# KoonMing/KZG-Batch-Verification-Scheme

Hardware: AMD Instinct MI355X
Metric: batch-verifies/sec + G1 MSM pts/sec at n=2^20, BLS12-381; 1/2/4/8 GPU (higher is better)
Workload: dtype Montgomery Fp, 381-bit modular integer (radix-2^29 limbs in the bucket accumulation); 1 GPU; batch_verify (configs[2]): n=1048576 bls12_381 tuples per GPU, two G1 MSMs + 2-pairing check; curve=bls12_381, tuples_per_gpu=1048576, global_batch=1048576, pipeline_slots=16, parallelism=point-range shards

## Files before the change

kzg-batch-verification-scheme_amd/csrc/field29.hpp:

```cpp
#pragma once
#include "field.hpp"
#include <type_traits>
#include "params29_gen.hpp"

namespace kzgmi {

constexpr uint32_t M29 = (1u << 29) - 1;

template <class Cv>
using Fp29Of = std::conditional_t<Cv::ID == 0, Bls12_381Fp29, Bn254Fp29>;

template <class Q>
struct F29 {
  static constexpr int N = Q::N;
  uint32_t v[N];
  KZ_DEV static F29 zero() { F29 r; _Pragma("unroll") for (int i = 0; i < N; ++i) r.v[i] = 0; return r; }
  KZ_DEV static F29 from_const(const uint32_t (&c)[N]) {
    F29 r;
    _Pragma("unroll") for (int i = 0; i < N; ++i) r.v[i] = c[i];
    return r;
  }
};

KZ_DEV void mad29(uint64_t& acc, uint32_t a, uint32_t b) {
// ... 197 lines not shown
      r.v[i] = x & M29;
      c = x >> 29;
    } else {
      r.v[i] = x;
    }
  }
  return r;
}

template <class Q>
KZ_DEV F29<Q> sub3_29(const F29<Q>& a, const F29<Q>& s, const F29<Q>& t, const uint32_t (&C)[Q::N]) {
  F29<Q> r;
  uint32_t c = 0;
  _Pragma("unroll") for (int i = 0; i < Q::N; ++i) {
    const uint32_t x = (a.v[i] + C[i] + c) - (s.v[i] + t.v[i] + t.v[i]);
    if (i < Q::N - 1) {
      r.v[i] = x & M29;
      c = x >> 29;
    } else {
      r.v[i] = x;
    }
  }
  return r;
}

template <class Q>
KZ_DEV F29<Q> neg_lazy29(const F29<Q>& b, const uint32_t (&B)[Q::N]) {
  F29<Q> r;
  _Pragma("unroll") for (int i = 0; i < Q::N; ++i) r.v[i] = B[i] - b.v[i];
  return r;
}

template <class Q>
KZ_DEV F29<Q> add3_29(const F29<Q>& a, const F29<Q>& b, const F29<Q>& e) {
  F29<Q> r;
  uint32_t c = 0;
  _Pragma("unroll") for (int i = 0; i < Q::N; ++i) {
    const uint32_t x = a.v[i] + b.v[i] + e.v[i] + c;
    if (i < Q::N - 1) {
      r.v[i] = x & M29;
      c = x >> 29;
    } else {
      r.v[i] = x;
    }
  }
  return r;
}

template <class Q>
KZ_DEV bool is_zero29(const F29<Q>& a) {
  bool hit = false;
  _Pragma("unroll") for (int k = 0; k < Q::NKP; ++k) hit |= a.v[0] == Q::KP_LO[k];
  if (!hit) return false;
  for (int k = 0; k < Q::NKP; ++k) {
    uint32_t d = 0;
    for (int i = 0; i < Q::N; ++i) d |= a.v[i] ^ Q::KP[k][i];
    if (d == 0) return true;
  }
  return false;
}
template <class Q>
KZ_DEV bool is_zero29_mf(const F29<Q>& a) {
  constexpr uint32_t PINV = 0u - Q::INV;
  const uint32_t k = (a.v[0] * PINV) & M29;
  if (k >= (uint32_t)Q::NKP) return false;
  uint32_t d = 0;
  for (int i = 0; i < Q::N; ++i) d |= a.v[i] ^ Q::KP[k][i];
  return d == 0;
}

template <class Q>
KZ_DEV F29<Q> canon29(const F29<Q>& a) {
  F29<Q> d;
  int32_t c = 0;
  _Pragma("unroll") for (int i = 0; i < Q::N; ++i) {
    const int32_t x = (int32_t)a.v[i] - (int32_t)Q::MOD[i] + c;
    if (i < Q::N - 1) {
      d.v[i] = (uint32_t)x & M29;
      c = x >> 29;
    } else {
      d.v[i] = (uint32_t)x;
    }
  }
  const bool neg = (int32_t)d.v[Q::N - 1] < 0;
  F29<Q> r;
  _Pragma("unroll") for (int i = 0; i < Q::N; ++i) r.v[i] = neg ? a.v[i] : d.v[i];
  return r;
}

template <class Q, int NW>
KZ_DEV F29<Q> limbs29(const uint32_t (&w)[NW]) {
  F29<Q> r;
  _Pragma("unroll") for (int i = 0; i < Q::N; ++i) {
    const int bit = 29 * i, wi = bit >> 5, sh = bit & 31;
    const uint64_t lo = (wi < NW ? (uint64_t)w[wi] : 0) | (wi + 1 < NW ? (uint64_t)w[wi + 1] << 32 : 0);
    r.v[i] = (uint32_t)(lo >> sh) & (i < Q::N - 1 ? M29 : 0xffffffffu);
  }
  return r;
}
template <class Q, int NW>
KZ_DEV void words32(const F29<Q>& a, uint32_t (&w)[NW]) {
  _Pragma("unroll") for (int j = 0; j < NW; ++j) {
    const int bit = 32 * j, li = bit / 29, sh = bit % 29;
    uint64_t x = (uint64_t)a.v[li] >> sh;
    if (li + 1 < Q::N) x |= (uint64_t)a.v[li + 1] << (29 - sh);
    if (li + 2 < Q::N && 58 - sh < 32) x |= (uint64_t)a.v[li + 2] << (58 - sh);
    w[j] = (uint32_t)x;
  }
}

template <class Q, class P>
KZ_DEV F29<Q> fp_to29(const Fp<P>& a) {
  return mul29(limbs29<Q>(a.v), F29<Q>::from_const(Q::TO29));
}
template <class Q, class P>
KZ_DEV Fp<P> fp_from29(const F29<Q>& a) {
  Fp<P> r;
  words32<Q>(canon29(mul29(a, F29<Q>::from_const(Q::TO32))), r.v);
  return r;
}

}
// ... 1 lines not shown
```

kzg-batch-verification-scheme_amd/csrc/launch_msm.hip:

```cpp
#include "launch.hpp"

namespace kzgmi {

template <class F>
void with_wbits(int wbits, F&& f) {
  if (wbits == 13) f(std::integral_constant<int, 13>{});
  else f(std::integral_constant<int, WBITS>{});
}

template <class Cv>
void Launch<Cv>::sort(hipStream_t st, const TermList& tl, uint32_t nsets, const uint8_t* inf, uint32_t* digits,
                      uint32_t* coarse, uint64_t* ent, size_t emax, int sort_flags, uint32_t* off, uint32_t* cnt, uint32_t* total, uint32_t* sval,
                      uint32_t* skey, int wbits) {
  const bool force_split = (sort_flags & SORT_SPLIT) != 0;
  with_wbits(wbits, [&](auto wb) {
    constexpr int WB = decltype(wb)::value;
    const uint32_t nbins = nsets * Win<WB>::BINS;
    SetShift ss;
    const bool table = !(sort_flags & SORT_FULL_BINS) && set_shifts_host<WB>(tl, nsets, ss);
    uint32_t* ccnt = coarse;
    uint32_t* coff = coarse + nbins;
    uint32_t* ccur = coarse + 2 * nbins;
    (void)hipMemsetAsync(ccnt, 0, (size_t)nbins * 4, st);
    const uint32_t tiles = num_tiles_host(tl);
// ... 20 lines not shown
  });
}

template <class Cv>
void Launch<Cv>::accumulate(hipStream_t st, size_t nchunks, const uint32_t* total, const uint32_t* sval,
                            const uint32_t* skey, const uint32_t* off, const uint32_t* cnt, const AF* pts,
                            uint32_t* acc29, uint32_t nb, size_t acc_threads, uint32_t* next_chunk,
                            uint32_t* crowd, const uint32_t* lo, hipStream_t fix_st) {
  const unsigned blocks = grid_for(nchunks, 256);
  if (next_chunk && acc_threads && acc_threads < nchunks) {
    (void)hipMemsetAsync(next_chunk, 0, 4, st);
    k_accumulate<Cv><<<grid_for(acc_threads, 256), 256, 0, st>>>(total, sval, skey, off, cnt, pts, acc29, nb,
                                                                  (uint32_t)(blocks * 256u), next_chunk, lo, crowd);
  } else {
    k_accumulate<Cv><<<blocks, 256, 0, st>>>(total, sval, skey, off, cnt, pts, acc29, nb, 0u, nullptr, lo, crowd);
  }
  if (fix_st) fixup(fix_st, nchunks, total, skey, off, cnt, acc29, nb, crowd, lo);
}

template <class Cv>
void Launch<Cv>::fixup(hipStream_t st, size_t nchunks, const uint32_t* total, const uint32_t* skey, const uint32_t* off,
                       const uint32_t* cnt, uint32_t* acc29, uint32_t nb, uint32_t* crowd, const uint32_t* lo) {
  const unsigned blocks = grid_for(nchunks, 256);
  k_fixup<Cv><<<blocks, 256, 0, st>>>(total, skey, off, cnt, acc29, nb, crowd, lo);
  k_fixup_crowded<Cv><<<256, 256, 0, st>>>(crowd, acc29, nb, blocks * 256u);
}

template <class Cv>
void Launch<Cv>::row_items(hipStream_t st, const uint32_t* off, const uint32_t* cnt, uint32_t nb, uint32_t L, uint32_t* rowq,
                           uint32_t* items, uint32_t cap, uint32_t* cuts, uint32_t cut_cap) {
  (void)hipMemsetAsync(rowq, 0, (size_t)RQ_WORDS * 4, st);
  const unsigned blocks = grid_for(nb, ITEMS_BLOCK);
  k_items_hist<<<blocks, 256, 0, st>>>(cnt, nb, L, rowq);
  k_items_scan<<<1, 256, 0, st>>>(L, rowq);
  k_items_scatter<<<blocks, 256, 0, st>>>(off, cnt, nb, L, rowq, items, cap, cuts, cut_cap);
}

template <class Cv>
void Launch<Cv>::accumulate_rows(hipStream_t st, size_t threads, const uint32_t* sval, const AF* pts, uint32_t* acc29,
                                 uint32_t nb, uint32_t* rowq, const uint32_t* items, uint32_t cap, const uint32_t* cuts,
                                 uint32_t cut_cap) {
  k_accumulate_rows<Cv><<<grid_for(threads, 256), 256, 0, st>>>(rowq, items, cap, sval, pts, acc29);
  k_join_rows<Cv><<<64, 256, 0, st>>>(rowq, cuts, acc29, nb, cut_cap);
}

template <class Cv>
void Launch<Cv>::pts_to29(hipStream_t st, AF* pts, uint32_t n) {
  if (n) k_pts_to29<Cv><<<grid_for(n, 256), 256, 0, st>>>(pts, n);
}

template <class Cv>
void Launch<Cv>::reduce(hipStream_t st, uint32_t nsets, const uint32_t* cnt, const uint32_t* acc29, XY* R, XY* U,
                        XY* scratch, XY* winsum, int wbits, bool low_prio, int seg4_waves, int simds) {
  with_wbits(wbits, [&](auto wb) {
    constexpr int WB = decltype(wb)::value;
    const uint32_t nseg = nsets * Win<WB>::NSEG;
    const bool four = seg4_waves > 0 && (size_t)nseg * 4 <= (size_t)seg4_waves * simds * 64;
    auto go = [&](auto lp) {
      constexpr bool LP = decltype(lp)::value;
      if (four) k_reduce_segments4<Cv, LP><<<grid_for(4 * (size_t)nseg, 256), 256, 0, st>>>(nseg, cnt, acc29, R, U);
      else k_reduce_segments<Cv, LP><<<grid_for(2 * (size_t)nseg, 256), 256, 0, st>>>(nseg, cnt, acc29, R, U);
      k_reduce_bits<Cv, WB, LP><<<nsets * Win<WB>::RB_PARTS, 256, 0, st>>>(R, U, scratch);
      if (four) k_reduce_bits_finish<Cv, WB, LP, 4><<<nsets, 64, 0, st>>>(scratch, winsum);
      else k_reduce_bits_finish<Cv, WB, LP, 2><<<nsets, 64, 0, st>>>(scratch, winsum);
    };
    if (low_prio) go(std::true_type{});
    else go(std::false_type{});
// ... 52 lines not shown
```

kzg-batch-verification-scheme_amd/csrc/msm.hpp:

```cpp
#pragma once
#include "common.hpp"
#include "field29.hpp"
#include "lpfield.hpp"

namespace kzgmi {

constexpr int WBITS = 16;
constexpr int NBUCKETS = 1 << (WBITS - 1);
constexpr int ACC_CHUNK = 64;
constexpr int ACC_CHUNK_SMALL = 16;
constexpr size_t ACC_SMALL_ENTRIES = size_t(1) << 20;
constexpr int SEG = 16;
constexpr int MAX_CLASSES = 16;

struct TermClass {
  uint32_t count;
  uint32_t pt_base;
  uint32_t scal_words;
  uint32_t nwin;
  uint32_t set_base;
  uint32_t scal_stride;
  const uint32_t* scal;
  uint32_t win_off;
  uint32_t dig_base;
// ... 632 lines not shown
  uint32_t w[W29];
#pragma unroll
  for (int k = 0; k < N; ++k) {
    w[k] = a.x.v[k];
    w[N + k] = a.y.v[k];
    w[2 * N + k] = a.inf ? 0u : a.zz.v[k];
    w[3 * N + k] = a.zzz.v[k];
  }
  uint4* d4 = reinterpret_cast<uint4*>(acc29 + r * W29);
#pragma unroll
  for (int k = 0; k < W29 / 4; ++k) d4[k] = make_uint4(w[4 * k], w[4 * k + 1], w[4 * k + 2], w[4 * k + 3]);
}
template <class Q>
KZ_DEV X29<Q> x29_swap_pair(const X29<Q>& a) {
  X29<Q> o;
#pragma unroll
  for (int k = 0; k < Q::N; ++k) {
    o.x.v[k] = (uint32_t)__shfl_xor((int)a.x.v[k], 1);
    o.y.v[k] = (uint32_t)__shfl_xor((int)a.y.v[k], 1);
    o.zz.v[k] = (uint32_t)__shfl_xor((int)a.zz.v[k], 1);
    o.zzz.v[k] = (uint32_t)__shfl_xor((int)a.zzz.v[k], 1);
  }
  o.inf = __shfl_xor((int)a.inf, 1) != 0;
  return o;
}
template <class Cv, class Q>
KZ_DEV Xyzz<Cv> x29_to32(const X29<Q>& a) {
  using P = typename Cv::FpP;
  if (a.inf) return Xyzz<Cv>::inf();
  return {fp_from29<Q, P>(a.x), fp_from29<Q, P>(a.y), fp_from29<Q, P>(a.zz), fp_from29<Q, P>(a.zzz)};
}
template <class Cv>
constexpr bool kFusedSub = Cv::ID == 0;

template <class Q>
KZ_DEV X29<Q> x29_dbl(const X29<Q>& a) {
  using G = F29<Q>;
  if (a.inf) return a;
  const G U = add3_29(a.y, a.y, G::zero());
  const G V = sqr29(U);
  const G W = mul29(U, V);
  const G S = mul29(a.x, V);
  const G X2 = sqr29(a.x);
  const G M = add3_29(X2, X2, X2);
  X29<Q> o;
  o.x = sub29(sqr29(M), add3_29(S, S, G::zero()), Q::B4);
  o.y = mul2_29(M, sub29(S, o.x, Q::B8), W, sub29(G::zero(), a.y, Q::B16));
  o.zz = mul29(V, a.zz);
  o.zzz = mul29(W, a.zzz);
  o.inf = false;
  return o;
}

template <class Cv, class Q>
KZ_DEV X29<Q> x29_add(const X29<Q>& a, const X29<Q>& b) {
  using G = F29<Q>;
  if (a.inf) return b;
  if (b.inf) return a;
  const G U1 = mul29(a.x, b.zz), S1 = mul29(a.y, b.zzz);
  const G P = kFusedSub<Cv> ? mulsub29(b.x, a.zz, U1, Q::B2) : sub29(mul29(b.x, a.zz), U1, Q::B2);
  const G R = kFusedSub<Cv> ? mulsub29(b.y, a.zzz, S1, Q::B2) : sub29(mul29(b.y, a.zzz), S1, Q::B2);
  if (is_zero29(P)) {
    if (is_zero29(R)) return x29_dbl<Q>(a);
    return {G::zero(), G::zero(), G::zero(), G::zero(), true};
  }
  const G PP = sqr29(P);
// ... 315 lines not shown
constexpr uint32_t ROW_LEN_MAX = 256;
enum : uint32_t {
  RQ_NEXT = 0, RQ_NITEMS = 1, RQ_NCUT = 2, RQ_PIECES = 3, RQ_HIST = 4, RQ_CUR = RQ_HIST + ROW_LEN_MAX + 1,
  RQ_WORDS = RQ_CUR + ROW_LEN_MAX + 1
};

KZ_DEV void items_count(uint32_t* h, uint32_t c, uint32_t L) {
  if (c <= L) {
    atomicAdd(&h[c], 1u);
  } else {
    atomicAdd(&h[L], c / L);
    if (c % L) atomicAdd(&h[c % L], 1u);
  }
}

constexpr uint32_t ITEMS_PER_THREAD = 4, ITEMS_BLOCK = 256 * ITEMS_PER_THREAD;

static __global__ void __launch_bounds__(256) k_items_hist(const uint32_t* __restrict__ cnt, uint32_t nb, uint32_t L,
                                                           uint32_t* __restrict__ rowq) {
  __shared__ uint32_t h[ROW_LEN_MAX + 1];
  for (uint32_t t = threadIdx.x; t <= L; t += blockDim.x) h[t] = 0;
  __syncthreads();
#pragma unroll
  for (uint32_t k = 0; k < ITEMS_PER_THREAD; ++k) {
    const uint32_t b = blockIdx.x * ITEMS_BLOCK + k * 256 + threadIdx.x;
    const uint32_t c = b < nb ? cnt[b] : 0u;
    if (c) items_count(h, c, L);
  }
  __syncthreads();
  for (uint32_t t = threadIdx.x; t <= L; t += blockDim.x)
    if (h[t]) atomicAdd(&rowq[RQ_HIST + t], h[t]);
}

static __global__ void __launch_bounds__(256) k_items_scan(uint32_t L, uint32_t* __restrict__ rowq) {
  __shared__ uint32_t h[ROW_LEN_MAX + 1];
  for (uint32_t t = threadIdx.x; t <= L; t += blockDim.x) h[t] = t ? rowq[RQ_HIST + t] : 0u;
  __syncthreads();
  for (uint32_t t = threadIdx.x; t <= L; t += blockDim.x) {
    uint32_t before = 0;
    for (uint32_t l = t + 1; l <= L; ++l) before += h[l];
    rowq[RQ_CUR + t] = before;
    if (t == 0) rowq[RQ_NITEMS] = before;
  }
}

static __global__ void __launch_bounds__(256) k_items_scatter(const uint32_t* __restrict__ off,
                                                              const uint32_t* __restrict__ cnt, uint32_t nb, uint32_t L,
                                                              uint32_t* __restrict__ rowq, uint32_t* __restrict__ items,
                                                              uint32_t cap, uint32_t* __restrict__ cuts, uint32_t cut_cap) {
  __shared__ uint32_t h[ROW_LEN_MAX + 1], base[ROW_LEN_MAX + 1];
  for (uint32_t t = threadIdx.x; t <= L; t += blockDim.x) h[t] = 0;
  __syncthreads();
  uint32_t c[ITEMS_PER_THREAD], rank[ITEMS_PER_THREAD];
#pragma unroll
  for (uint32_t k = 0; k < ITEMS_PER_THREAD; ++k) {
    const uint32_t b = blockIdx.x * ITEMS_BLOCK + k * 256 + threadIdx.x;
    c[k] = b < nb ? cnt[b] : 0u;
    rank[k] = c[k] && c[k] <= L ? atomicAdd(&h[c[k]], 1u) : 0u;
  }
  __syncthreads();
  for (uint32_t t = threadIdx.x; t <= L; t += blockDim.x)
    if (h[t]) base[t] = atomicAdd(&rowq[RQ_CUR + t], h[t]);
  __syncthreads();
  auto put = [&](uint32_t pos, uint32_t rec, uint32_t first, uint32_t len) {
    if (pos >= cap) return;
    items[pos] = rec;
    items[cap + pos] = first;
    items[2 * (size_t)cap + pos] = len;
  };
#pragma unroll
  for (uint32_t k = 0; k < ITEMS_PER_THREAD; ++k) {
    const uint32_t b = blockIdx.x * ITEMS_BLOCK + k * 256 + threadIdx.x;
    if (!c[k]) continue;
    const uint32_t o = off[b];
    if (c[k] <= L) {
      put(base[c[k]] + rank[k], b, o, c[k]);
      continue;
    }
    const uint32_t np = (c[k] + L - 1) / L;
    const uint32_t slot = atomicAdd(&rowq[RQ_PIECES], np);
    const uint32_t line = atomicAdd(&rowq[RQ_NCUT], 1u);
    if (line >= cut_cap) continue;
    cuts[3 * (size_t)line] = b;
    cuts[3 * (size_t)line + 1] = slot;
    cuts[3 * (size_t)line + 2] = np;
    for (uint32_t j = 0; j < np; ++j) {
      const uint32_t len = min(L, c[k] - j * L);
      put(atomicAdd(&rowq[RQ_CUR + len], 1u), nb + slot + j, o + j * L, len);
    }
  }
}

template <class Cv>
KZ_DEV void acc_row29(uint32_t first, uint32_t len, uint32_t rec, const uint32_t* __restrict__ sorted_val,
                      const uint32_t* __restrict__ pts29, uint32_t* __restrict__ acc29) {
  using Q = Fp29Of<Cv>;
  using G = F29<Q>;
  constexpr int N = Q::N, W29 = kW29<Q>;
  __shared__ uint32_t s_zz[N][256], s_zzz[N][256];
  __shared__ uint4 s_vq[256];
  const uint32_t tx = threadIdx.x;
  auto ld = [tx](uint32_t (&a)[N][256]) {
    asm volatile("" ::: "memory");
    G r;
    _Pragma("unroll") for (int k = 0; k < N; ++k) r.v[k] = a[k][tx];
    return r;
  };
  auto st = [tx](uint32_t (&a)[N][256], const G& v) {
    _Pragma("unroll") for (int k = 0; k < N; ++k) a[k][tx] = v.v[k];
    asm volatile("" ::: "memory");
  };
  auto put = [](uint32_t* d, const G& a) {
    if constexpr (N % 2 == 0) {
      _Pragma("unroll") for (int k = 0; k < N / 2; ++k) reinterpret_cast<uint2*>(d)[k] = make_uint2(a.v[2 * k], a.v[2 * k + 1]);
    } else {
      _Pragma("unroll") for (int k = 0; k < N; ++k) d[k] = a.v[k];
    }
  };
  auto load_q = [&](uint32_t v, G& qx, G& qy) {
    load_pt29<Cv>(reinterpret_cast<const Affine<Cv>*>(pts29) + sv_point(v), qx, qy);
    if (v & 1) qy = sub29(G::zero(), qy, Q::ACC_NEG);
  };
  auto set_one = [&]() {
    const G one = one_literals<Q>(std::make_integer_sequence<int, N / 2>{});
    st(s_zz, one);
    st(s_zzz, one);
  };
  uint4* const vq_wave = &s_vq[tx & ~63u];
  const uint32_t end = first + len;
  uint32_t e = first;
  G x, y;
  bool inf = false;
  load_q(sorted_val[e], x, y);
  set_one();
  ++e;
  for (;;) {
    bool dbl = false;
    __builtin_amdgcn_global_load_lds(reinterpret_cast<const uint4*>(sorted_val + (e & ~3u)), vq_wave, 16, 0, 0);
    for (; e < end; ++e) {
      const uint32_t j = e & 3u;
      uint32_t lane;
      asm volatile("v_mbcnt_lo_u32_b32 %0, -1, 0\n\tv_mbcnt_hi_u32_b32 %0, -1, %0" : "=v"(lane));
      const uint32_t v = reinterpret_cast<const uint32_t*>(&s_vq[(tx & ~63u) + lane])[j];
      if (j == 3) {
        __builtin_amdgcn_s_waitcnt(0xc07f);
        __builtin_amdgcn_global_load_lds(reinterpret_cast<const uint4*>(sorted_val + e + 1), vq_wave, 16, 0, 0);
      }
      G qx, qy;
      load_q(v, qx, qy);
      if (inf) {
        x = qx;
        y = qy;
        set_one();
        inf = false;
        continue;
      }
      const G P = kFusedSub<Cv> ? mulsub29(qx, ld(s_zz), x, Q::ACC_P) : sub29(mul29(qx, ld(s_zz)), x, Q::ACC_P);
      const G R = kFusedSub<Cv> ? mulsub29(qy, ld(s_zzz), y, Q::ACC_R) : sub29(mul29(qy, ld(s_zzz)), y, Q::ACC_R);
      if (is_zero29_mf(P)) {
        if (is_zero29_mf(R)) {
          dbl = true;
          break;
        }
        inf = true;
        continue;
      }
      const G PP = sqr29(P);
      const G PPP = mul29(P, PP);
      st(s_zz, mul29(ld(s_zz), PP));
      st(s_zzz, mul29(ld(s_zzz), PPP));
      const G Q2 = mul29(x, PP);
      const G X3 = kFusedSub<Cv> ? sqrsub3_29(R, PPP, Q2, Q::ACC_X3) : sub3_29(sqr29(R), PPP, Q2, Q::ACC_X3);
      y = mul2_29(R, sub29(Q2, X3, Q::ACC_QX), y, neg_lazy29(PPP, Q::ACC_PPP));
      x = X3;
    }
    if (!dbl) break;
    G qx, qy;
    load_q(sorted_val[e], qx, qy);
    asm volatile("" ::: "memory");
    const Xy29<Q> d = dbl_affine29<Q>(qx, qy, &s_zz[0][tx], &s_zzz[0][tx]);
    asm volatile("" ::: "memory");
    x = d.x;
    y = d.y;
    ++e;
  }
  uint32_t* d = acc29 + (size_t)rec * W29;
  put(d, x);
  put(d + N, y);
  put(d + 2 * N, inf ? G::zero() : ld(s_zz));
  put(d + 3 * N, ld(s_zzz));
}

template <class Cv>
__global__ void __launch_bounds__(256) __attribute__((amdgpu_waves_per_eu(kAccWaves<Cv>))) k_accumulate_rows(
    uint32_t* __restrict__ rowq, const uint32_t* __restrict__ items, uint32_t cap,
    const uint32_t* __restrict__ sorted_val, const Affine<Cv>* __restrict__ pts, uint32_t* __restrict__ acc29) {
  const uint32_t nitems = rowq[RQ_NITEMS];
  const uint32_t lane = threadIdx.x & 63u;
  for (;;) {
    uint32_t row = 0;
    if (lane == 0) row = atomicAdd(&rowq[RQ_NEXT], 1u);
    row = __shfl(row, 0);
    if ((uint64_t)row * 64 >= nitems) break;
    const uint32_t i = row * 64 + lane;
    if (i < nitems)
      acc_row29<Cv>(items[cap + i], items[2 * (size_t)cap + i], items[i], sorted_val,
                    reinterpret_cast<const uint32_t*>(pts), acc29);
  }
}

template <class Cv>
// ... 318 lines not shown
```

kzg-batch-verification-scheme_amd/csrc/params29_gen.hpp:

```cpp
#pragma once
#include <cstdint>

namespace kzgmi {

struct Bls12_381Fp29 {
  static constexpr int N = 14;
  static constexpr uint32_t MOD[N] = {0x1fffaaabu, 0xff7ffffu, 0x14ffffeeu, 0x17fffd62u, 0xf6241eau, 0x9507b58u, 0xafd9cc3u, 0x109e70a2u, 0x1764774bu, 0x121a5d66u, 0x12c6e9edu, 0x12ffcd34u, 0x111ea3u, 0xdu};
  static constexpr uint32_t INV = 0xfffcfffdu;
  static constexpr uint32_t ONE[N] = {0x3a9fb84u, 0xba00690u, 0x71288f1u, 0xf59bcc5u, 0x126cb614u, 0x585bf36u, 0x1b85ac3du, 0x1cf856fau, 0x1891ecbdu, 0x1a7eec05u, 0x155a88f0u, 0x741ac6du, 0x1317c30fu, 0x9u};
  static constexpr uint32_t TO29[N] = {0x1fddebbdu, 0x1a4f5474u, 0x291f399u, 0x14d03b3cu, 0xf6cad2cu, 0x1b4cabcau, 0x1592827cu, 0x21c6ac7u, 0x1ec52a84u, 0x16fd5ec4u, 0xc960da6u, 0xfd2af6bu, 0x13263591u, 0xbu};
  static constexpr uint32_t TO32[N] = {0x2fffdu, 0x10480000u, 0x300009du, 0x8001788u, 0x158baebfu, 0xc2ba9e3u, 0x1d157d22u, 0xa6e0a4au, 0xd77ce58u, 0x1d12b763u, 0x1701c6a5u, 0x1501c926u, 0x1f65ec3fu, 0xau};
  static constexpr uint32_t R2[N] = {0x15bef7aeu, 0x1031cd0eu, 0x2dd93e8u, 0x9226323u, 0xe6e2cd2u, 0x11684daau, 0x1170e5dbu, 0x88e25b1u, 0x1b366399u, 0x1c536f47u, 0xd1f9cbcu, 0x278b67fu, 0x1ea66a2bu, 0xcu};
  static constexpr uint32_t BCURVE[N] = {0xea898bau, 0xe901a40u, 0x124a23e8u, 0xd66f84fu, 0xaee547cu, 0x3760629u, 0x181b776eu, 0x12a47aa6u, 0x137ec460u, 0x5c6f549u, 0xfdc4fe8u, 0x1707174du, 0xc3ccef5u, 0xcu};
  static constexpr uint32_t B1[N] = {0x3fffaaabu, 0x2ff7fffeu, 0x34ffffedu, 0x37fffd61u, 0x2f6241e9u, 0x29507b57u, 0x2afd9cc2u, 0x309e70a1u, 0x3764774au, 0x321a5d65u, 0x32c6e9ecu, 0x32ffcd33u, 0x20111ea2u, 0xcu};
  static constexpr uint32_t B2[N] = {0x3fff5556u, 0x3feffffeu, 0x29ffffdbu, 0x2ffffac4u, 0x3ec483d4u, 0x32a0f6afu, 0x35fb3985u, 0x213ce143u, 0x2ec8ee96u, 0x2434baccu, 0x258dd3dau, 0x25ff9a68u, 0x20223d46u, 0x19u};
  static constexpr uint32_t B4[N] = {0x3ffeaaacu, 0x3fdffffeu, 0x33ffffb8u, 0x3ffff589u, 0x3d8907a9u, 0x2541ed60u, 0x2bf6730cu, 0x2279c288u, 0x3d91dd2du, 0x28697599u, 0x2b1ba7b5u, 0x2bff34d1u, 0x20447a8du, 0x33u};
  static constexpr uint32_t B8[N] = {0x3ffd5558u, 0x3fbffffeu, 0x27ffff72u, 0x3fffeb14u, 0x3b120f54u, 0x2a83dac2u, 0x37ece619u, 0x24f38511u, 0x3b23ba5bu, 0x30d2eb34u, 0x36374f6bu, 0x37fe69a3u, 0x2088f51bu, 0x67u};
  static constexpr uint32_t B16[N] = {0x3ffaaab0u, 0x3f7ffffeu, 0x2ffffee6u, 0x3fffd629u, 0x36241eaau, 0x3507b586u, 0x2fd9cc33u, 0x29e70a24u, 0x364774b7u, 0x21a5d66au, 0x2c6e9ed8u, 0x2ffcd348u, 0x2111ea38u, 0xcfu};
  static constexpr uint32_t B32[N] = {0x3ff55560u, 0x3efffffeu, 0x3ffffdceu, 0x3fffac53u, 0x2c483d56u, 0x2a0f6b0eu, 0x3fb39868u, 0x33ce1449u, 0x2c8ee96fu, 0x234bacd6u, 0x38dd3db1u, 0x3ff9a691u, 0x2223d471u, 0x19fu};
  static constexpr uint32_t B64[N] = {0x3feaaac0u, 0x3dfffffeu, 0x3ffffb9eu, 0x3fff58a8u, 0x38907aaeu, 0x341ed61du, 0x3f6730d1u, 0x279c2894u, 0x391dd2e0u, 0x269759adu, 0x31ba7b63u, 0x3ff34d24u, 0x2447a8e4u, 0x33fu};
  static constexpr uint32_t C4[N] = {0x7ffeaaacu, 0x7fdffffcu, 0x73ffffb6u, 0x7ffff587u, 0x7d8907a7u, 0x6541ed5eu, 0x6bf6730au, 0x6279c286u, 0x7d91dd2bu, 0x68697597u, 0x6b1ba7b3u, 0x6bff34cfu, 0x60447a8bu, 0x31u};
  static constexpr uint32_t C8[N] = {0x7ffd5558u, 0x7fbffffcu, 0x67ffff70u, 0x7fffeb12u, 0x7b120f52u, 0x6a83dac0u, 0x77ece617u, 0x64f3850fu, 0x7b23ba59u, 0x70d2eb32u, 0x76374f69u, 0x77fe69a1u, 0x6088f519u, 0x65u};
  static constexpr const uint32_t (&ACC_NEG)[N] = B8;
  static constexpr const uint32_t (&ACC_P)[N] = B16;
  static constexpr const uint32_t (&ACC_R)[N] = B16;
  static constexpr const uint32_t (&ACC_X3)[N] = C8;
  static constexpr const uint32_t (&ACC_QX)[N] = B16;
  static constexpr const uint32_t (&ACC_PPP)[N] = B8;
  static constexpr const uint32_t (&DBL_X)[N] = B8;
  static constexpr const uint32_t (&DBL_QX)[N] = B16;
  static constexpr const uint32_t (&DBL_Y)[N] = B8;
  static constexpr const uint32_t (&ACC_X3_B)[N] = B8;
  static constexpr int NKP = 20;
  static constexpr uint32_t KP_LO[NKP] = {0x0u, 0x1fffaaabu, 0x1fff5556u, 0x1fff0001u, 0x1ffeaaacu, 0x1ffe5557u, 0x1ffe0002u, 0x1ffdaaadu, 0x1ffd5558u, 0x1ffd0003u, 0x1ffcaaaeu, 0x1ffc5559u, 0x1ffc0004u, 0x1ffbaaafu, 0x1ffb555au, 0x1ffb0005u, 0x1ffaaab0u, 0x1ffa555bu, 0x1ffa0006u, 0x1ff9aab1u};
  static constexpr uint32_t KP[NKP][N] = {{0x0u, 0x0u, 0x0u, 0x0u, 0x0u, 0x0u, 0x0u, 0x0u, 0x0u, 0x0u, 0x0u, 0x0u, 0x0u, 0x0u}, {0x1fffaaabu, 0xff7ffffu, 0x14ffffeeu, 0x17fffd62u, 0xf6241eau, 0x9507b58u, 0xafd9cc3u, 0x109e70a2u, 0x1764774bu, 0x121a5d66u, 0x12c6e9edu, 0x12ffcd34u, 0x111ea3u, 0xdu}, {0x1fff5556u, 0x1fefffffu, 0x9ffffdcu, 0xffffac5u, 0x1ec483d5u, 0x12a0f6b0u, 0x15fb3986u, 0x13ce144u, 0xec8ee97u, 0x434bacdu, 0x58dd3dbu, 0x5ff9a69u, 0x223d47u, 0x1au}, {0x1fff0001u, 0xfe7ffffu, 0x1effffcbu, 0x7fff827u, 0xe26c5c0u, 0x1bf17209u, 0xf8d649u, 0x11db51e7u, 0x62d65e2u, 0x164f1834u, 0x1854bdc8u, 0x18ff679du, 0x335beau, 0x27u}, {0x1ffeaaacu, 0x1fdfffffu, 0x13ffffb9u, 0x1ffff58au, 0x1d8907aau, 0x541ed61u, 0xbf6730du, 0x279c289u, 0x1d91dd2eu, 0x869759au, 0xb1ba7b6u, 0xbff34d2u, 0x447a8eu, 0x34u}, {0x1ffe5557u, 0xfd7ffffu, 0x8ffffa8u, 0x17fff2edu, 0xceb4995u, 0xe9268bau, 0x16f40fd0u, 0x1318332bu, 0x14f65479u, 0x1a83d301u, 0x1de291a3u, 0x1eff0206u, 0x559931u, 0x41u}, {0x1ffe0002u, 0x1fcfffffu, 0x1dffff96u, 0xffff04fu, 0x1c4d8b80u, 0x17e2e412u, 0x1f1ac93u, 0x3b6a3ceu, 0xc5acbc5u, 0xc9e3068u, 0x10a97b91u, 0x11fecf3bu, 0x66b7d5u, 0x4eu}, {0x1ffdaaadu, 0xfc7ffffu, 0x12ffff85u, 0x7ffedb2u, 0xbafcd6bu, 0x1335f6bu, 0xcef4957u, 0x14551470u, 0x3bf4310u, 0x1eb88dcfu, 0x370657eu, 0x4fe9c70u, 0x77d679u, 0x5bu}, {0x1ffd5558u, 0x1fbfffffu, 0x7ffff73u, 0x1fffeb15u, 0x1b120f55u, 0xa83dac3u, 0x17ece61au, 0x4f38512u, 0x1b23ba5cu, 0x10d2eb35u, 0x16374f6cu, 0x17fe69a4u, 0x88f51cu, 0x68u}, {0x1ffd0003u, 0xfb7ffffu, 0x1cffff62u, 0x17ffe877u, 0xa745140u, 0x13d4561cu, 0x2ea82ddu, 0x1591f5b5u, 0x128831a7u, 0x2ed489cu, 0x8fe395au, 0xafe36d9u, 0x9a13c0u, 0x75u}, {0x1ffcaaaeu, 0x1fafffffu, 0x11ffff50u, 0xfffe5dau, 0x19d6932bu, 0x1d24d174u, 0xde81fa0u, 0x6306657u, 0x9eca8f3u, 0x1507a603u, 0x1bc52347u, 0x1dfe040du, 0xab3263u, 0x82u}, {0x1ffc5559u, 0xfa7ffffu, 0x6ffff3fu, 0x7ffe33du, 0x938d516u, 0x6754ccdu, 0x18e5bc64u, 0x16ced6f9u, 0x151203eu, 0x722036au, 0xe8c0d35u, 0x10fdd142u, 0xbc5107u, 0x8fu}, {0x1ffc0004u, 0x1f9fffffu, 0x1bffff2du, 0x1fffe09fu, 0x189b1700u, 0xfc5c825u, 0x3e35927u, 0x76d479cu, 0x18b5978au, 0x193c60d0u, 0x152f722u, 0x3fd9e77u, 0xcd6fabu, 0x9cu}, {0x1ffbaaafu, 0xf97ffffu, 0x10ffff1cu, 0x17ffde02u, 0x7fd58ebu, 0x1916437eu, 0xee0f5eau, 0x180bb83eu, 0x101a0ed5u, 0xb56be37u, 0x1419e110u, 0x16fd6babu, 0xde8e4eu, 0xa9u}, {0x1ffb555au, 0x1f8fffffu, 0x5ffff0au, 0xfffdb65u, 0x175f9ad6u, 0x266bed6u, 0x19de92aeu, 0x8aa28e0u, 0x77e8621u, 0x1d711b9eu, 0x6e0cafdu, 0x9fd38e0u, 0xefacf2u, 0xb6u}, {0x1ffb0005u, 0xf87ffffu, 0x1afffef9u, 0x7ffd8c7u, 0x6c1dcc1u, 0xbb73a2fu, 0x4dc2f71u, 0x19489983u, 0x1ee2fd6cu, 0xf8b7904u, 0x19a7b4ebu, 0x1cfd0614u, 0x100cb95u, 0xc3u}, {0x1ffaaab0u, 0x1f7fffffu, 0xffffee7u, 0x1fffd62au, 0x16241eabu, 0x1507b587u, 0xfd9cc34u, 0x9e70a25u, 0x164774b8u, 0x1a5d66bu, 0xc6e9ed9u, 0xffcd349u, 0x111ea39u, 0xd0u}, {0x1ffa555bu, 0xf77ffffu, 0x4fffed6u, 0x17ffd38du, 0x5866096u, 0x1e5830e0u, 0x1ad768f7u, 0x1a857ac7u, 0xdabec03u, 0x13c033d2u, 0x1f3588c6u, 0x2fca07du, 0x12308ddu, 0xddu}, {0x1ffa0006u, 0x1f6fffffu, 0x19fffec4u, 0xfffd0efu, 0x14e8a281u, 0x7a8ac38u, 0x5d505bbu, 0xb23eb6au, 0x510634fu, 0x5da9139u, 0x11fc72b4u, 0x15fc6db2u, 0x1342780u, 0xeau}, {0x1ff9aab1u, 0xf67ffffu, 0xefffeb3u, 0x7ffce52u, 0x44ae46cu, 0x10f92791u, 0x10d2a27eu, 0x1bc25c0cu, 0x1c74da9au, 0x17f4ee9fu, 0x4c35ca1u, 0x8fc3ae7u, 0x1454624u, 0xf7u}};
};

struct Bn254Fp29 {
  static constexpr int N = 9;
  static constexpr uint32_t MOD[N] = {0x187cfd47u, 0x10460b6u, 0x1c72a34fu, 0x2d522d0u, 0x1585d978u, 0x2db40c0u, 0xa6e141u, 0xe5c2634u, 0x30644eu};
  static constexpr uint32_t INV = 0xe4866389u;
  static constexpr uint32_t ONE[N] = {0x157ccc21u, 0x141c2758u, 0x185230d3u, 0x14c0419u, 0xaa36fb9u, 0x1d4240ceu, 0x11d54c07u, 0x52ac7a8u, 0xdc836u};
  static constexpr uint32_t TO29[N] = {0x13349ca1u, 0x1a5d84a8u, 0xa3e5cacu, 0x100249e0u, 0x12b951e8u, 0xe92d304u, 0x14cb95b3u, 0x41b9d3du, 0x58003u};
  static constexpr uint32_t TO32[N] = {0x58f0d9du, 0x1aea1c6eu, 0x11c2cf74u, 0x11d651ebu, 0x1462c0a7u, 0x11b7bc3cu, 0x1cbd99bau, 0x183340fbu, 0xe0a77u};
  static constexpr uint32_t R2[N] = {0x59bac10u, 0xd1503a3u, 0x18016b8u, 0x10ab0ca8u, 0x2632639u, 0x2c0169fu, 0x169bfd53u, 0x11869d4cu, 0x2a11a6u};
  static constexpr uint32_t BCURVE[N] = {0x766463u, 0x1c54760au, 0x8f6927au, 0x3e40c4du, 0x1fea4f2bu, 0x17c6c26au, 0x157fe417u, 0xf8056f9u, 0x2958a2u};
  static constexpr uint32_t B1[N] = {0x387cfd47u, 0x210460b5u, 0x3c72a34eu, 0x22d522cfu, 0x3585d977u, 0x22db40bfu, 0x20a6e140u, 0x2e5c2633u, 0x30644du};
  static constexpr uint32_t B2[N] = {0x30f9fa8eu, 0x2208c16cu, 0x38e5469du, 0x25aa45a0u, 0x2b0bb2efu, 0x25b68180u, 0x214dc281u, 0x3cb84c67u, 0x60c89bu};
  static constexpr uint32_t B4[N] = {0x21f3f51cu, 0x241182dau, 0x31ca8d3bu, 0x2b548b42u, 0x361765dfu, 0x2b6d0301u, 0x229b8503u, 0x397098cfu, 0xc19138u};
  static constexpr uint32_t B8[N] = {0x23e7ea38u, 0x282305b5u, 0x23951a77u, 0x36a91686u, 0x2c2ecbbfu, 0x36da0604u, 0x25370a07u, 0x32e1319fu, 0x1832272u};
  static constexpr uint32_t B16[N] = {0x27cfd470u, 0x30460b6bu, 0x272a34efu, 0x2d522d0du, 0x385d9780u, 0x2db40c09u, 0x2a6e1410u, 0x25c2633fu, 0x30644e6u};
  static constexpr uint32_t B32[N] = {0x2f9fa8e0u, 0x208c16d7u, 0x2e5469e0u, 0x3aa45a1bu, 0x30bb2f01u, 0x3b681814u, 0x34dc2821u, 0x2b84c67fu, 0x60c89cdu};
  static constexpr uint32_t B64[N] = {0x3f3f51c0u, 0x21182dafu, 0x3ca8d3c1u, 0x3548b437u, 0x21765e04u, 0x36d0302au, 0x29b85044u, 0x37098d00u, 0xc19139bu};
  static constexpr uint32_t C4[N] = {0x61f3f51cu, 0x641182d8u, 0x71ca8d39u, 0x6b548b40u, 0x761765ddu, 0x6b6d02ffu, 0x629b8501u, 0x797098cdu, 0xc19136u};
  static constexpr uint32_t C8[N] = {0x63e7ea38u, 0x682305b3u, 0x63951a75u, 0x76a91684u, 0x6c2ecbbdu, 0x76da0602u, 0x65370a05u, 0x72e1319du, 0x1832270u};
  static constexpr const uint32_t (&ACC_NEG)[N] = B2;
  static constexpr const uint32_t (&ACC_P)[N] = B8;
  static constexpr const uint32_t (&ACC_R)[N] = B4;
  static constexpr const uint32_t (&ACC_X3)[N] = C4;
  static constexpr const uint32_t (&ACC_QX)[N] = B8;
  static constexpr const uint32_t (&ACC_PPP)[N] = B2;
  static constexpr const uint32_t (&DBL_X)[N] = B4;
  static constexpr const uint32_t (&DBL_QX)[N] = B8;
  static constexpr const uint32_t (&DBL_Y)[N] = B2;
  static constexpr const uint32_t (&ACC_X3_B)[N] = B4;
// ... 7 lines not shown
```

Before: 199.7 batch-verifies/s (n=1048576 tuples per GPU per batch).

## Peel first bucket addition, use lazy negation, fold item scan into scatter

In BLS12-381 bucket row accumulation, the first two points of a row are now added with a specialised affine+affine step. It is guarded by range checks on the top limbs and a wave-wide ballot, so the generic mixed add and the set_one store are skipped when the inputs are safe. Point negation in the main loop uses a lazy unreduced form, normalised only when it is loaded into an infinity accumulator. The separate single-block k_items_scan launch is removed: every scatter block recomputes the suffix sums in shared memory and adds them to its atomic offsets. This trades redundant per-block scan work and extra range-check logic for one fewer kernel launch and less field arithmetic.

```diff
diff --git a/kzg-batch-verification-scheme_amd/csrc/field29.hpp b/kzg-batch-verification-scheme_amd/csrc/field29.hpp
--- a/kzg-batch-verification-scheme_amd/csrc/field29.hpp
+++ b/kzg-batch-verification-scheme_amd/csrc/field29.hpp
@@ -253,6 +253,22 @@
 }
 
 template <class Q>
+KZ_DEV F29<Q> norm29(const F29<Q>& a) {
+  F29<Q> r;
+  uint32_t c = 0;
+  _Pragma("unroll") for (int i = 0; i < Q::N; ++i) {
+    const uint32_t x = a.v[i] + c;
+    if (i < Q::N - 1) {
+      r.v[i] = x & M29;
+      c = x >> 29;
+    } else {
+      r.v[i] = x;
+    }
+  }
+  return r;
+}
+
+template <class Q>
 KZ_DEV F29<Q> add3_29(const F29<Q>& a, const F29<Q>& b, const F29<Q>& e) {
   F29<Q> r;
   uint32_t c = 0;
@@ -309,6 +325,15 @@
   return r;
 }
 
+template <class Q>
+KZ_DEV bool peel_ok29(const F29<Q>& v) {
+  constexpr int N = Q::N;
+  const uint32_t t1 = v.v[N - 1], t0 = v.v[N - 2];
+  const bool lo = (t1 != 0) | (t0 >= Q::PEEL_LO);
+  const bool hi = (t1 < Q::MOD[N - 1]) | ((t1 == Q::MOD[N - 1]) & (t0 < Q::MOD[N - 2]));
+  return lo & hi;
+}
+
 template <class Q, int NW>
 KZ_DEV F29<Q> limbs29(const uint32_t (&w)[NW]) {
   F29<Q> r;
diff --git a/kzg-batch-verification-scheme_amd/csrc/launch_msm.hip b/kzg-batch-verification-scheme_amd/csrc/launch_msm.hip
--- a/kzg-batch-verification-scheme_amd/csrc/launch_msm.hip
+++ b/kzg-batch-verification-scheme_amd/csrc/launch_msm.hip
@@ -76,7 +76,6 @@
   (void)hipMemsetAsync(rowq, 0, (size_t)RQ_WORDS * 4, st);
   const unsigned blocks = grid_for(nb, ITEMS_BLOCK);
   k_items_hist<<<blocks, 256, 0, st>>>(cnt, nb, L, rowq);
-  k_items_scan<<<1, 256, 0, st>>>(L, rowq);
   k_items_scatter<<<blocks, 256, 0, st>>>(off, cnt, nb, L, rowq, items, cap, cuts, cut_cap);
 }
 
diff --git a/kzg-batch-verification-scheme_amd/csrc/msm.hpp b/kzg-batch-verification-scheme_amd/csrc/msm.hpp
--- a/kzg-batch-verification-scheme_amd/csrc/msm.hpp
+++ b/kzg-batch-verification-scheme_amd/csrc/msm.hpp
@@ -688,6 +688,8 @@
 }
 template <class Cv>
 constexpr bool kFusedSub = Cv::ID == 0;
+template <class Cv>
+constexpr bool kPeelFirst = Cv::ID == 0;
 
 template <class Q>
 KZ_DEV X29<Q> x29_dbl(const X29<Q>& a) {
@@ -1069,25 +1071,22 @@
     if (h[t]) atomicAdd(&rowq[RQ_HIST + t], h[t]);
 }
 
-static __global__ void __launch_bounds__(256) k_items_scan(uint32_t L, uint32_t* __restrict__ rowq) {
-  __shared__ uint32_t h[ROW_LEN_MAX + 1];
-  for (uint32_t t = threadIdx.x; t <= L; t += blockDim.x) h[t] = t ? rowq[RQ_HIST + t] : 0u;
-  __syncthreads();
-  for (uint32_t t = threadIdx.x; t <= L; t += blockDim.x) {
-    uint32_t before = 0;
-    for (uint32_t l = t + 1; l <= L; ++l) before += h[l];
-    rowq[RQ_CUR + t] = before;
-    if (t == 0) rowq[RQ_NITEMS] = before;
-  }
-}
-
 static __global__ void __launch_bounds__(256) k_items_scatter(const uint32_t* __restrict__ off,
                                                               const uint32_t* __restrict__ cnt, uint32_t nb, uint32_t L,
                                                               uint32_t* __restrict__ rowq, uint32_t* __restrict__ items,
                                                               uint32_t cap, uint32_t* __restrict__ cuts, uint32_t cut_cap) {
-  __shared__ uint32_t h[ROW_LEN_MAX + 1], base[ROW_LEN_MAX + 1];
-  for (uint32_t t = threadIdx.x; t <= L; t += blockDim.x) h[t] = 0;
-  __syncthreads();
+  __shared__ uint32_t h[ROW_LEN_MAX + 1], base[ROW_LEN_MAX + 1], all[ROW_LEN_MAX + 1], before[ROW_LEN_MAX + 1];
+  for (uint32_t t = threadIdx.x; t <= L; t += blockDim.x) {
+    h[t] = 0;
+    all[t] = t ? rowq[RQ_HIST + t] : 0u;
+  }
+  __syncthreads();
+  for (uint32_t t = threadIdx.x; t <= L; t += blockDim.x) {
+    uint32_t s = 0;
+    for (uint32_t l = t + 1; l <= L; ++l) s += all[l];
+    before[t] = s;
+    if (t == 0 && blockIdx.x == 0) rowq[RQ_NITEMS] = s;
+  }
   uint32_t c[ITEMS_PER_THREAD], rank[ITEMS_PER_THREAD];
 #pragma unroll
   for (uint32_t k = 0; k < ITEMS_PER_THREAD; ++k) {
@@ -1097,7 +1096,7 @@
   }
   __syncthreads();
   for (uint32_t t = threadIdx.x; t <= L; t += blockDim.x)
-    if (h[t]) base[t] = atomicAdd(&rowq[RQ_CUR + t], h[t]);
+    if (h[t]) base[t] = before[t] + atomicAdd(&rowq[RQ_CUR + t], h[t]);
   __syncthreads();
   auto put = [&](uint32_t pos, uint32_t rec, uint32_t first, uint32_t len) {
     if (pos >= cap) return;
@@ -1123,7 +1122,7 @@
     cuts[3 * (size_t)line + 2] = np;
     for (uint32_t j = 0; j < np; ++j) {
       const uint32_t len = min(L, c[k] - j * L);
-      put(atomicAdd(&rowq[RQ_CUR + len], 1u), nb + slot + j, o + j * L, len);
+      put(before[len] + atomicAdd(&rowq[RQ_CUR + len], 1u), nb + slot + j, o + j * L, len);
     }
   }
 }
@@ -1154,10 +1153,15 @@
       _Pragma("unroll") for (int k = 0; k < N; ++k) d[k] = a.v[k];
     }
   };
-  auto load_q = [&](uint32_t v, G& qx, G& qy) {
+  auto load_q = [&](uint32_t v, G& qx, G& qy, auto lazy) {
     load_pt29<Cv>(reinterpret_cast<const Affine<Cv>*>(pts29) + sv_point(v), qx, qy);
-    if (v & 1) qy = sub29(G::zero(), qy, Q::ACC_NEG);
+    if (v & 1) {
+      if constexpr (decltype(lazy)::value) qy = neg_lazy29(qy, Q::ACC_NEG);
+      else qy = sub29(G::zero(), qy, Q::ACC_NEG);
+    }
   };
+  constexpr std::false_type normalised{};
+  constexpr std::true_type lazy_neg{};
   auto set_one = [&]() {
     const G one = one_literals<Q>(std::make_integer_sequence<int, N / 2>{});
     st(s_zz, one);
@@ -1168,9 +1172,42 @@
   uint32_t e = first;
   G x, y;
   bool inf = false;
-  load_q(sorted_val[e], x, y);
-  set_one();
+  load_q(sorted_val[e], x, y, normalised);
   ++e;
+  bool one = true;
+  if constexpr (kPeelFirst<Cv>) {
+    const bool two = e < end;
+    bool ok = true;
+    G R, PP, PPP;
+    if (two) {
+      const uint32_t v = sorted_val[e];
+      G qx, S2;
+      load_pt29<Cv>(reinterpret_cast<const Affine<Cv>*>(pts29) + sv_point(v), qx, S2);
+      if (v & 1) S2 = sub29(G::zero(), S2, Q::B1);
+      ok = peel_ok29(qx) & peel_ok29(S2);
+      const G P = sub29(qx, x, Q::ACC_P);
+      R = sub29(S2, y, Q::ACC_R);
+      ok &= !is_zero29_mf(P);
+      PP = sqr29(P);
+      const G zz = canon29(PP);
+      st(s_zz, zz);
+      PPP = mul29(P, PP);
+      const G zzz = canon29(PPP);
+      st(s_zzz, zzz);
+      ok &= peel_ok29(zz) & peel_ok29(zzz);
+    }
+    if (__ballot(two && !ok) == 0) {
+      if (two) {
+        const G Q2 = mul29(x, PP);
+        const G X3 = kFusedSub<Cv> ? sqrsub3_29(R, PPP, Q2, Q::ACC_X3) : sub3_29(sqr29(R), PPP, Q2, Q::ACC_X3);
+        y = mul2_29(R, sub29(Q2, X3, Q::ACC_QX), y, neg_lazy29(PPP, Q::ACC_PPP));
+        x = X3;
+        ++e;
+        one = false;
+      }
+    }
+  }
+  if (one) set_one();
   for (;;) {
     bool dbl = false;
     __builtin_amdgcn_global_load_lds(reinterpret_cast<const uint4*>(sorted_val + (e & ~3u)), vq_wave, 16, 0, 0);
@@ -1184,10 +1221,10 @@
         __builtin_amdgcn_global_load_lds(reinterpret_cast<const uint4*>(sorted_val + e + 1), vq_wave, 16, 0, 0);
       }
       G qx, qy;
-      load_q(v, qx, qy);
+      load_q(v, qx, qy, lazy_neg);
       if (inf) {
         x = qx;
-        y = qy;
+        y = norm29(qy);
         set_one();
         inf = false;
         continue;
@@ -1213,7 +1250,7 @@
     }
     if (!dbl) break;
     G qx, qy;
-    load_q(sorted_val[e], qx, qy);
+    load_q(sorted_val[e], qx, qy, normalised);
     asm volatile("" ::: "memory");
     const Xy29<Q> d = dbl_affine29<Q>(qx, qy, &s_zz[0][tx], &s_zzz[0][tx]);
     asm volatile("" ::: "memory");
diff --git a/kzg-batch-verification-scheme_amd/csrc/params29_gen.hpp b/kzg-batch-verification-scheme_amd/csrc/params29_gen.hpp
--- a/kzg-batch-verification-scheme_amd/csrc/params29_gen.hpp
+++ b/kzg-batch-verification-scheme_amd/csrc/params29_gen.hpp
@@ -31,6 +31,7 @@
   static constexpr const uint32_t (&DBL_QX)[N] = B16;
   static constexpr const uint32_t (&DBL_Y)[N] = B8;
   static constexpr const uint32_t (&ACC_X3_B)[N] = B8;
+  static constexpr uint32_t PEEL_LO = 999;
   static constexpr int NKP = 20;
   static constexpr uint32_t KP_LO[NKP] = {0x0u, 0x1fffaaabu, 0x1fff5556u, 0x1fff0001u, 0x1ffeaaacu, 0x1ffe5557u, 0x1ffe0002u, 0x1ffdaaadu, 0x1ffd5558u, 0x1ffd0003u, 0x1ffcaaaeu, 0x1ffc5559u, 0x1ffc0004u, 0x1ffbaaafu, 0x1ffb555au, 0x1ffb0005u, 0x1ffaaab0u, 0x1ffa555bu, 0x1ffa0006u, 0x1ff9aab1u};
   static constexpr uint32_t KP[NKP][N] = {{0x0u, 0x0u, 0x0u, 0x0u, 0x0u, 0x0u, 0x0u, 0x0u, 0x0u, 0x0u, 0x0u, 0x0u, 0x0u, 0x0u}, {0x1fffaaabu, 0xff7ffffu, 0x14ffffeeu, 0x17fffd62u, 0xf6241eau, 0x9507b58u, 0xafd9cc3u, 0x109e70a2u, 0x1764774bu, 0x121a5d66u, 0x12c6e9edu, 0x12ffcd34u, 0x111ea3u, 0xdu}, {0x1fff5556u, 0x1fefffffu, 0x9ffffdcu, 0xffffac5u, 0x1ec483d5u, 0x12a0f6b0u, 0x15fb3986u, 0x13ce144u, 0xec8ee97u, 0x434bacdu, 0x58dd3dbu, 0x5ff9a69u, 0x223d47u, 0x1au}, {0x1fff0001u, 0xfe7ffffu, 0x1effffcbu, 0x7fff827u, 0xe26c5c0u, 0x1bf17209u, 0xf8d649u, 0x11db51e7u, 0x62d65e2u, 0x164f1834u, 0x1854bdc8u, 0x18ff679du, 0x335beau, 0x27u}, {0x1ffeaaacu, 0x1fdfffffu, 0x13ffffb9u, 0x1ffff58au, 0x1d8907aau, 0x541ed61u, 0xbf6730du, 0x279c289u, 0x1d91dd2eu, 0x869759au, 0xb1ba7b6u, 0xbff34d2u, 0x447a8eu, 0x34u}, {0x1ffe5557u, 0xfd7ffffu, 0x8ffffa8u, 0x17fff2edu, 0xceb4995u, 0xe9268bau, 0x16f40fd0u, 0x1318332bu, 0x14f65479u, 0x1a83d301u, 0x1de291a3u, 0x1eff0206u, 0x559931u, 0x41u}, {0x1ffe0002u, 0x1fcfffffu, 0x1dffff96u, 0xffff04fu, 0x1c4d8b80u, 0x17e2e412u, 0x1f1ac93u, 0x3b6a3ceu, 0xc5acbc5u, 0xc9e3068u, 0x10a97b91u, 0x11fecf3bu, 0x66b7d5u, 0x4eu}, {0x1ffdaaadu, 0xfc7ffffu, 0x12ffff85u, 0x7ffedb2u, 0xbafcd6bu, 0x1335f6bu, 0xcef4957u, 0x14551470u, 0x3bf4310u, 0x1eb88dcfu, 0x370657eu, 0x4fe9c70u, 0x77d679u, 0x5bu}, {0x1ffd5558u, 0x1fbfffffu, 0x7ffff73u, 0x1fffeb15u, 0x1b120f55u, 0xa83dac3u, 0x17ece61au, 0x4f38512u, 0x1b23ba5cu, 0x10d2eb35u, 0x16374f6cu, 0x17fe69a4u, 0x88f51cu, 0x68u}, {0x1ffd0003u, 0xfb7ffffu, 0x1cffff62u, 0x17ffe877u, 0xa745140u, 0x13d4561cu, 0x2ea82ddu, 0x1591f5b5u, 0x128831a7u, 0x2ed489cu, 0x8fe395au, 0xafe36d9u, 0x9a13c0u, 0x75u}, {0x1ffcaaaeu, 0x1fafffffu, 0x11ffff50u, 0xfffe5dau, 0x19d6932bu, 0x1d24d174u, 0xde81fa0u, 0x6306657u, 0x9eca8f3u, 0x1507a603u, 0x1bc52347u, 0x1dfe040du, 0xab3263u, 0x82u}, {0x1ffc5559u, 0xfa7ffffu, 0x6ffff3fu, 0x7ffe33du, 0x938d516u, 0x6754ccdu, 0x18e5bc64u, 0x16ced6f9u, 0x151203eu, 0x722036au, 0xe8c0d35u, 0x10fdd142u, 0xbc5107u, 0x8fu}, {0x1ffc0004u, 0x1f9fffffu, 0x1bffff2du, 0x1fffe09fu, 0x189b1700u, 0xfc5c825u, 0x3e35927u, 0x76d479cu, 0x18b5978au, 0x193c60d0u, 0x152f722u, 0x3fd9e77u, 0xcd6fabu, 0x9cu}, {0x1ffbaaafu, 0xf97ffffu, 0x10ffff1cu, 0x17ffde02u, 0x7fd58ebu, 0x1916437eu, 0xee0f5eau, 0x180bb83eu, 0x101a0ed5u, 0xb56be37u, 0x1419e110u, 0x16fd6babu, 0xde8e4eu, 0xa9u}, {0x1ffb555au, 0x1f8fffffu, 0x5ffff0au, 0xfffdb65u, 0x175f9ad6u, 0x266bed6u, 0x19de92aeu, 0x8aa28e0u, 0x77e8621u, 0x1d711b9eu, 0x6e0cafdu, 0x9fd38e0u, 0xefacf2u, 0xb6u}, {0x1ffb0005u, 0xf87ffffu, 0x1afffef9u, 0x7ffd8c7u, 0x6c1dcc1u, 0xbb73a2fu, 0x4dc2f71u, 0x19489983u, 0x1ee2fd6cu, 0xf8b7904u, 0x19a7b4ebu, 0x1cfd0614u, 0x100cb95u, 0xc3u}, {0x1ffaaab0u, 0x1f7fffffu, 0xffffee7u, 0x1fffd62au, 0x16241eabu, 0x1507b587u, 0xfd9cc34u, 0x9e70a25u, 0x164774b8u, 0x1a5d66bu, 0xc6e9ed9u, 0xffcd349u, 0x111ea39u, 0xd0u}, {0x1ffa555bu, 0xf77ffffu, 0x4fffed6u, 0x17ffd38du, 0x5866096u, 0x1e5830e0u, 0x1ad768f7u, 0x1a857ac7u, 0xdabec03u, 0x13c033d2u, 0x1f3588c6u, 0x2fca07du, 0x12308ddu, 0xddu}, {0x1ffa0006u, 0x1f6fffffu, 0x19fffec4u, 0xfffd0efu, 0x14e8a281u, 0x7a8ac38u, 0x5d505bbu, 0xb23eb6au, 0x510634fu, 0x5da9139u, 0x11fc72b4u, 0x15fc6db2u, 0x1342780u, 0xeau}, {0x1ff9aab1u, 0xf67ffffu, 0xefffeb3u, 0x7ffce52u, 0x44ae46cu, 0x10f92791u, 0x10d2a27eu, 0x1bc25c0cu, 0x1c74da9au, 0x17f4ee9fu, 0x4c35ca1u, 0x8fc3ae7u, 0x1454624u, 0xf7u}};
```

Result: faster. 202.1 batch-verifies/s (n=1048576 tuples per GPU per batch) (median of 6 runs) (+1.2%).
